# svip-lab/impersonator

Measured on NVIDIA H100. Metric: frames/sec @256x256 (per-frame inference hot path), higher is better.
Workload: dtype f16 main product + e4m3 correction products (hi/lo split), f32 accumulate

## Files before the change

impersonator_b200/csrc/conv_tc.cu:

```cuda
#include <cuda.h>

#include <stdlib.h>

#include <algorithm>
#include <new>
#include <type_traits>

#include "common.cuh"

namespace {

constexpr int TILE_H = 16, TILE_W = 8;
constexpr int SWAP_N_TILE = 64;
constexpr int SWAP_TILE_H = 32;
constexpr int KCHUNK = 64;
constexpr int ROW_BYTES = TILE_W * 128;
constexpr int MAX_TAPS = 49;
constexpr int MAX_GROUP = 8;
constexpr int RING_BYTES = 200 * 1024;
constexpr int MAX_STAGES = 8;
constexpr int NUM_CONSUMERS = 256;
constexpr int NUM_THREADS = NUM_CONSUMERS + 128;
constexpr int MAX_N_TILE = 128;
static_assert(2 * 2 * (TILE_H + MAX_GROUP - 1) * ROW_BYTES + 2 * 2 * MAX_N_TILE * 128 <= RING_BYTES,
              "every plan needs two A and two B entries in the ring");
static_assert(2 * 2 * (SWAP_TILE_H + MAX_GROUP - 1) * ROW_BYTES + 2 * 2 * SWAP_N_TILE * 128 <= RING_BYTES,
              "every swapped plan needs two A and two B entries in the ring");
static_assert(SWAP_N_TILE * (SWAP_TILE_H * TILE_W) == MAX_N_TILE * (TILE_H * TILE_W), "same accumulator budget");

__host__ __device__ constexpr int tile_rows(int n_tile) { return n_tile == SWAP_N_TILE ? SWAP_TILE_H : TILE_H; }

struct ConvParams {
    CUtensorMap a_hi[4];
    CUtensorMap a_lo[4];
    CUtensorMap w_hi;
    CUtensorMap w_lo;
    int n_img, tiles_y, tiles_x, n_tiles_n;
    int dom_h, dom_w;
    int ntaps, chunks0, chunks1;
    signed char dy[MAX_TAPS], dx[MAX_TAPS], tmap[MAX_TAPS];
    short wtap[MAX_TAPS];
    int ngroups;
    signed char g_first[MAX_TAPS], g_cnt[MAX_TAPS];
    int a_rows;
    int a_stages, b_stages;
    float* out; int out_h, out_w, cout;
    int oy_mul, oy_add, ox_mul, ox_add;
    double* stats;
    float out_scale;
    int phase_cols;
};

template <int N_TILE, bool SPLIT>
struct Cfg {
    static constexpr int B_BYTES = N_TILE * 128;
    static constexpr int B_STAGE_BYTES = B_BYTES * (SPLIT ? 2 : 1);
    static constexpr int BAR_BYTES = 4 * MAX_STAGES * 8;
    static constexpr int STATS_PARTS = N_TILE < SWAP_N_TILE ? 8 : N_TILE == SWAP_N_TILE ? 2 : 0;
    static constexpr int STATS_BYTES = STATS_PARTS * N_TILE * 8;
    static constexpr int SMEM_BYTES = 1024 + RING_BYTES + BAR_BYTES + STATS_BYTES;
    static_assert(B_STAGE_BYTES % 1024 == 0, "B entries must keep the 1024-byte swizzle alignment");
    static_assert(SMEM_BYTES <= 227 * 1024, "exceeds the shared memory of a block");
};

__device__ __forceinline__ uint32_t smem_u32(const void* p) { return (uint32_t)__cvta_generic_to_shared(p); }

__device__ __forceinline__ void mbar_init(uint64_t* bar, uint32_t count) {
    asm volatile("mbarrier.init.shared::cta.b64 [%0], %1;" ::"r"(smem_u32(bar)), "r"(count));
}
__device__ __forceinline__ void mbar_expect_tx(uint64_t* bar, uint32_t bytes) {
    asm volatile("mbarrier.arrive.expect_tx.shared::cta.b64 _, [%0], %1;" ::"r"(smem_u32(bar)), "r"(bytes) : "memory");
}
__device__ __forceinline__ void mbar_arrive(uint64_t* bar) {
    asm volatile("mbarrier.arrive.shared::cta.b64 _, [%0];" ::"r"(smem_u32(bar)) : "memory");
}
__device__ __forceinline__ bool mbar_try_wait(uint64_t* bar, uint32_t parity) {
    uint32_t ok;
    asm volatile("{\n\t.reg .pred p;\n\t"
                 "mbarrier.try_wait.parity.shared::cta.b64 p, [%1], %2;\n\t"
                 "selp.u32 %0, 1, 0, p;\n\t}"
                 : "=r"(ok) : "r"(smem_u32(bar)), "r"(parity) : "memory");
    return ok != 0;
}
__device__ __forceinline__ void mbar_wait(uint64_t* bar, uint32_t parity) {
    if (mbar_try_wait(bar, parity)) return;
    const long long t0 = clock64();
    while (!mbar_try_wait(bar, parity)) {
        if (clock64() - t0 > 4000000000ll) __trap();
    }
}
__device__ __forceinline__ bool elect_one() {
    uint32_t pred;
    asm volatile("{\n\t.reg .pred P;\n\telect.sync _|P, 0xffffffff;\n\tselp.b32 %0, 1, 0, P;\n\t}" : "=r"(pred));
    return pred != 0;
}
__device__ __forceinline__ void fence_barrier_init() { asm volatile("fence.mbarrier_init.release.cluster;" ::: "memory"); }
__device__ __forceinline__ void fence_proxy_async() { asm volatile("fence.proxy.async.shared::cta;" ::: "memory"); }

__device__ __forceinline__ void tma_load_4d(const CUtensorMap* map, void* dst, uint64_t* bar, int c0, int c1, int c2, int c3) {
    asm volatile("cp.async.bulk.tensor.4d.shared::cluster.global.mbarrier::complete_tx::bytes [%0], [%1, {%3, %4, %5, %6}], [%2];"
                 :: "r"(smem_u32(dst)), "l"(map), "r"(smem_u32(bar)), "r"(c0), "r"(c1), "r"(c2), "r"(c3) : "memory");
}
__device__ __forceinline__ void tma_load_3d(const CUtensorMap* map, void* dst, uint64_t* bar, int c0, int c1, int c2) {
    asm volatile("cp.async.bulk.tensor.3d.shared::cluster.global.mbarrier::complete_tx::bytes [%0], [%1, {%3, %4, %5}], [%2];"
                 :: "r"(smem_u32(dst)), "l"(map), "r"(smem_u32(bar)), "r"(c0), "r"(c1), "r"(c2) : "memory");
}

__device__ __forceinline__ uint64_t make_desc(uint32_t smem_addr) {
    return (uint64_t)((smem_addr & 0x3FFFF) >> 4) | (1ull << 16) | (64ull << 32) | (1ull << 62);
}
__device__ __forceinline__ void wgmma_fence() { asm volatile("wgmma.fence.sync.aligned;" ::: "memory"); }
__device__ __forceinline__ void wgmma_commit() { asm volatile("wgmma.commit_group.sync.aligned;" ::: "memory"); }
template <int N>
__device__ __forceinline__ void wgmma_wait() { asm volatile("wgmma.wait_group.sync.aligned %0;" :: "n"(N) : "memory"); }
__device__ __forceinline__ void acc_fence(float& r) { asm volatile("" : "+f"(r) :: "memory"); }

template <int N> __device__ __forceinline__ void wgmma_f16(float* d, uint64_t da, uint64_t db);
template <int N> __device__ __forceinline__ void wgmma_e4m3(float* d, uint64_t da, uint64_t db);
template <> __device__ __forceinline__ void wgmma_f16<16>(float* d, uint64_t da, uint64_t db) {
    asm volatile("{\n\t.reg .pred p;\n\tsetp.ne.b32 p, %10, 0;\n\t"
                 "wgmma.mma_async.sync.aligned.m64n16k16.f32.f16.f16 {%0, %1, %2, %3, %4, %5, %6, %7}, %8, %9, p, 1, 1, 0, 0;\n\t}"
                 : "+f"(d[0]), "+f"(d[1]), "+f"(d[2]), "+f"(d[3]), "+f"(d[4]), "+f"(d[5]), "+f"(d[6]), "+f"(d[7])
                 : "l"(da), "l"(db), "r"(1));
}
template <> __device__ __forceinline__ void wgmma_f16<32>(float* d, uint64_t da, uint64_t db) {
    asm volatile("{\n\t.reg .pred p;\n\tsetp.ne.b32 p, %18, 0;\n\t"
                 "wgmma.mma_async.sync.aligned.m64n32k16.f32.f16.f16 {%0, %1, %2, %3, %4, %5, %6, %7, %8, %9, %10, %11, %12, %13, %14, %15}, %16, %17, p, 1, 1, 0, 0;\n\t}"
                 : "+f"(d[0]), "+f"(d[1]), "+f"(d[2]), "+f"(d[3]), "+f"(d[4]), "+f"(d[5]), "+f"(d[6]), "+f"(d[7]), "+f"(d[8]), "+f"(d[9]), "+f"(d[10]), "+f"(d[11]), "+f"(d[12]), "+f"(d[13]), "+f"(d[14]), "+f"(d[15])
                 : "l"(da), "l"(db), "r"(1));
}
template <> __device__ __forceinline__ void wgmma_f16<128>(float* d, uint64_t da, uint64_t db) {
    asm volatile("{\n\t.reg .pred p;\n\tsetp.ne.b32 p, %66, 0;\n\t"
                 "wgmma.mma_async.sync.aligned.m64n128k16.f32.f16.f16 {%0, %1, %2, %3, %4, %5, %6, %7, %8, %9, %10, %11, %12, %13, %14, %15, %16, %17, %18, %19, %20, %21, %22, %23, %24, %25, %26, %27, %28, %29, %30, %31, %32, %33, %34, %35, %36, %37, %38, %39, %40, %41, %42, %43, %44, %45, %46, %47, %48, %49, %50, %51, %52, %53, %54, %55, %56, %57, %58, %59, %60, %61, %62, %63}, %64, %65, p, 1, 1, 0, 0;\n\t}"
                 : "+f"(d[0]), "+f"(d[1]), "+f"(d[2]), "+f"(d[3]), "+f"(d[4]), "+f"(d[5]), "+f"(d[6]), "+f"(d[7]), "+f"(d[8]), "+f"(d[9]), "+f"(d[10]), "+f"(d[11]), "+f"(d[12]), "+f"(d[13]), "+f"(d[14]), "+f"(d[15]), "+f"(d[16]), "+f"(d[17]), "+f"(d[18]), "+f"(d[19]), "+f"(d[20]), "+f"(d[21]), "+f"(d[22]), "+f"(d[23]), "+f"(d[24]), "+f"(d[25]), "+f"(d[26]), "+f"(d[27]), "+f"(d[28]), "+f"(d[29]), "+f"(d[30]), "+f"(d[31]), "+f"(d[32]), "+f"(d[33]), "+f"(d[34]), "+f"(d[35]), "+f"(d[36]), "+f"(d[37]), "+f"(d[38]), "+f"(d[39]), "+f"(d[40]), "+f"(d[41]), "+f"(d[42]), "+f"(d[43]), "+f"(d[44]), "+f"(d[45]), "+f"(d[46]), "+f"(d[47]), "+f"(d[48]), "+f"(d[49]), "+f"(d[50]), "+f"(d[51]), "+f"(d[52]), "+f"(d[53]), "+f"(d[54]), "+f"(d[55]), "+f"(d[56]), "+f"(d[57]), "+f"(d[58]), "+f"(d[59]), "+f"(d[60]), "+f"(d[61]), "+f"(d[62]), "+f"(d[63])
                 : "l"(da), "l"(db), "r"(1));
}
template <> __device__ __forceinline__ void wgmma_e4m3<16>(float* d, uint64_t da, uint64_t db) {
    asm volatile("{\n\t.reg .pred p;\n\tsetp.ne.b32 p, %10, 0;\n\t"
                 "wgmma.mma_async.sync.aligned.m64n16k32.f32.e4m3.e4m3 {%0, %1, %2, %3, %4, %5, %6, %7}, %8, %9, p, 1, 1;\n\t}"
                 : "+f"(d[0]), "+f"(d[1]), "+f"(d[2]), "+f"(d[3]), "+f"(d[4]), "+f"(d[5]), "+f"(d[6]), "+f"(d[7])
                 : "l"(da), "l"(db), "r"(1));
}
template <> __device__ __forceinline__ void wgmma_e4m3<32>(float* d, uint64_t da, uint64_t db) {
    asm volatile("{\n\t.reg .pred p;\n\tsetp.ne.b32 p, %18, 0;\n\t"
                 "wgmma.mma_async.sync.aligned.m64n32k32.f32.e4m3.e4m3 {%0, %1, %2, %3, %4, %5, %6, %7, %8, %9, %10, %11, %12, %13, %14, %15}, %16, %17, p, 1, 1;\n\t}"
                 : "+f"(d[0]), "+f"(d[1]), "+f"(d[2]), "+f"(d[3]), "+f"(d[4]), "+f"(d[5]), "+f"(d[6]), "+f"(d[7]), "+f"(d[8]), "+f"(d[9]), "+f"(d[10]), "+f"(d[11]), "+f"(d[12]), "+f"(d[13]), "+f"(d[14]), "+f"(d[15])
                 : "l"(da), "l"(db), "r"(1));
}
template <> __device__ __forceinline__ void wgmma_e4m3<128>(float* d, uint64_t da, uint64_t db) {
    asm volatile("{\n\t.reg .pred p;\n\tsetp.ne.b32 p, %66, 0;\n\t"
                 "wgmma.mma_async.sync.aligned.m64n128k32.f32.e4m3.e4m3 {%0, %1, %2, %3, %4, %5, %6, %7, %8, %9, %10, %11, %12, %13, %14, %15, %16, %17, %18, %19, %20, %21, %22, %23, %24, %25, %26, %27, %28, %29, %30, %31, %32, %33, %34, %35, %36, %37, %38, %39, %40, %41, %42, %43, %44, %45, %46, %47, %48, %49, %50, %51, %52, %53, %54, %55, %56, %57, %58, %59, %60, %61, %62, %63}, %64, %65, p, 1, 1;\n\t}"
                 : "+f"(d[0]), "+f"(d[1]), "+f"(d[2]), "+f"(d[3]), "+f"(d[4]), "+f"(d[5]), "+f"(d[6]), "+f"(d[7]), "+f"(d[8]), "+f"(d[9]), "+f"(d[10]), "+f"(d[11]), "+f"(d[12]), "+f"(d[13]), "+f"(d[14]), "+f"(d[15]), "+f"(d[16]), "+f"(d[17]), "+f"(d[18]), "+f"(d[19]), "+f"(d[20]), "+f"(d[21]), "+f"(d[22]), "+f"(d[23]), "+f"(d[24]), "+f"(d[25]), "+f"(d[26]), "+f"(d[27]), "+f"(d[28]), "+f"(d[29]), "+f"(d[30]), "+f"(d[31]), "+f"(d[32]), "+f"(d[33]), "+f"(d[34]), "+f"(d[35]), "+f"(d[36]), "+f"(d[37]), "+f"(d[38]), "+f"(d[39]), "+f"(d[40]), "+f"(d[41]), "+f"(d[42]), "+f"(d[43]), "+f"(d[44]), "+f"(d[45]), "+f"(d[46]), "+f"(d[47]), "+f"(d[48]), "+f"(d[49]), "+f"(d[50]), "+f"(d[51]), "+f"(d[52]), "+f"(d[53]), "+f"(d[54]), "+f"(d[55]), "+f"(d[56]), "+f"(d[57]), "+f"(d[58]), "+f"(d[59]), "+f"(d[60]), "+f"(d[61]), "+f"(d[62]), "+f"(d[63])
                 : "l"(da), "l"(db), "r"(1));
}

__device__ __forceinline__ void consumer_sync() { asm volatile("bar.sync 1, 256;" ::: "memory"); }

struct TileCoord {
    int n_idx, img, y0, x0;
};
template <int TH>
__device__ __forceinline__ TileCoord decode_tile(const ConvParams& P, int tile, int m_tiles) {
    TileCoord t;
    t.n_idx = tile / m_tiles;
    const int m_idx = tile % m_tiles;
    t.img = m_idx / (P.tiles_y * P.tiles_x);
    const int rem = m_idx % (P.tiles_y * P.tiles_x);
    t.y0 = (rem / P.tiles_x) * TH; t.x0 = (rem % P.tiles_x) * TILE_W;
    return t;
}

template <int N_TILE>
__device__ __forceinline__ void warp_tile_stats(const float* acc, bool v0, bool v1, int warp, unsigned lane, float2* s_stats)
{
#pragma unroll
    for (int j = 0; j < N_TILE / 8; j++) {
        const float a0 = v0 ? acc[4 * j] : 0.f, a1 = v0 ? acc[4 * j + 1] : 0.f;
        const float b0 = v1 ? acc[4 * j + 2] : 0.f, b1 = v1 ? acc[4 * j + 3] : 0.f;
        float s0 = a0 + b0, s1 = a1 + b1, q0 = a0 * a0 + b0 * b0, q1 = a1 * a1 + b1 * b1;
#pragma unroll
        for (int off = 4; off <= 16; off <<= 1) {
            s0 += __shfl_xor_sync(0xffffffffu, s0, off); s1 += __shfl_xor_sync(0xffffffffu, s1, off);
            q0 += __shfl_xor_sync(0xffffffffu, q0, off); q1 += __shfl_xor_sync(0xffffffffu, q1, off);
        }
        if (lane < 4) {
            s_stats[warp * N_TILE + 8 * j + 2 * lane] = make_float2(s0, q0);
            s_stats[warp * N_TILE + 8 * j + 2 * lane + 1] = make_float2(s1, q1);
        }
    }
}

template <int N_TILE, int PARTS>
__device__ __forceinline__ void flush_tile_stats(const ConvParams& P, const float2* s_stats, int img, int n_idx)
{
    consumer_sync();
    for (int col = threadIdx.x; col < N_TILE; col += NUM_CONSUMERS) {
        float s = 0.f, q = 0.f;
#pragma unroll
        for (int w = 0; w < PARTS; w++) { const float2 v = s_stats[w * N_TILE + col]; s += v.x; q += v.y; }
        int ch = n_idx * N_TILE + col;
        if (P.phase_cols > 0) ch %= P.phase_cols;
        double* dst = P.stats + 2 * ((size_t)img * P.cout + ch);
        atomicAdd(dst, (double)s);
        atomicAdd(dst + 1, (double)q);
    }
    consumer_sync();
}

template <int N_TILE>
__device__ __forceinline__ void epilogue_plain(const ConvParams& P, float* acc, const TileCoord& t, int warp, unsigned lane,
                                               float2* s_stats)
{
    const int tx = (int)(lane >> 2), x = t.x0 + tx;
    const int y[2] = {t.y0 + 2 * warp, t.y0 + 2 * warp + 1};
    const bool valid[2] = {y[0] < P.dom_h && x < P.dom_w, y[1] < P.dom_h && x < P.dom_w};
    if (P.out_scale != 1.f) {
#pragma unroll
        for (int i = 0; i < N_TILE / 2; i++) acc[i] *= P.out_scale;
    }
    if (P.out) {
        const int out_w_c = P.out_w * P.cout;
#pragma unroll
        for (int h = 0; h < 2; h++) {
            if (!valid[h]) continue;
            float* optr = P.out + (((size_t)t.img * P.out_h + (P.oy_mul * y[h] + P.oy_add)) * P.out_w + (P.ox_mul * x + P.ox_add)) * P.cout
                        + (size_t)t.n_idx * N_TILE;
#pragma unroll
            for (int j = 0; j < N_TILE / 8; j++) {
                const int c = 8 * j + 2 * (int)(lane & 3);
                float* o = optr + c;
                if (P.phase_cols > 0) {
                    const int col = t.n_idx * N_TILE + c, ph = col / P.phase_cols;
                    o = P.out + (((size_t)t.img * P.out_h + 2 * y[h]) * P.out_w + 2 * x) * P.cout
                      + (size_t)(ph >> 1) * out_w_c + (ph & 1) * P.cout + (col - ph * P.phase_cols);
                }
                *reinterpret_cast<float2*>(o) = make_float2(acc[4 * j + 2 * h], acc[4 * j + 2 * h + 1]);
            }
        }
    }
    if (P.stats) {
        warp_tile_stats<N_TILE>(acc, valid[0], valid[1], warp, lane, s_stats);
        flush_tile_stats<N_TILE, 8>(P, s_stats, t.img, t.n_idx);
    }
}

template <int N_TILE>
__device__ __forceinline__ void epilogue_channel_major(const ConvParams& P, float* acc, const TileCoord& t, int warp,
                                                       unsigned lane, float2* s_stats)
{
    const int wg = warp >> 2;
    const int c_base = N_TILE == MAX_N_TILE ? 64 * wg : 0, row0 = N_TILE == MAX_N_TILE ? 0 : 16 * wg;
    const int c0 = c_base + 16 * (warp & 3) + (int)(lane >> 2);
    const int y0 = t.y0 + row0, x0 = t.x0 + 2 * (int)(lane & 3);
    const int rows = P.dom_h - y0;
    const bool vx[2] = {x0 < P.dom_w, x0 + 1 < P.dom_w};
    const int col = t.n_idx * N_TILE + c0;
    const int ph = P.phase_cols > 0 ? col / P.phase_cols : 0;
    const int ch = col - ph * P.phase_cols;
    const size_t coff = ((size_t)(ph >> 1) * P.out_w + (ph & 1)) * P.cout + ch;
    if (P.out_scale != 1.f) {
#pragma unroll
        for (int i = 0; i < 64; i++) acc[i] *= P.out_scale;
    }
    if (P.out) {
#pragma unroll
        for (int j = 0; j < 16; j++) {
            if (j >= rows) break;
            const size_t orow = ((size_t)t.img * P.out_h + (P.oy_mul * (y0 + j) + P.oy_add)) * P.out_w;
#pragma unroll
            for (int e = 0; e < 2; e++) {
                if (!vx[e]) continue;
                float* o = P.out + (orow + (P.ox_mul * (x0 + e) + P.ox_add)) * P.cout;
                o[coff] = acc[4 * j + e];
                o[coff + 8] = acc[4 * j + 2 + e];
            }
        }
    }
    if (P.stats) {
        float s[2] = {0.f, 0.f}, q[2] = {0.f, 0.f};
#pragma unroll
        for (int j = 0; j < 16; j++) {
#pragma unroll
            for (int e = 0; e < 2; e++) {
                const bool v = j < rows && vx[e];
#pragma unroll
                for (int h = 0; h < 2; h++) {
                    const float a = v ? acc[4 * j + 2 * h + e] : 0.f;
                    s[h] += a; q[h] += a * a;
                }
            }
        }
#pragma unroll
        for (int h = 0; h < 2; h++) {
#pragma unroll
            for (int off = 1; off <= 2; off <<= 1) {
                s[h] += __shfl_xor_sync(0xffffffffu, s[h], off);
                q[h] += __shfl_xor_sync(0xffffffffu, q[h], off);
            }
        }
        if constexpr (N_TILE == SWAP_N_TILE) {
            if ((lane & 3) == 0) {
                s_stats[wg * N_TILE + c0] = make_float2(s[0], q[0]);
                s_stats[wg * N_TILE + c0 + 8] = make_float2(s[1], q[1]);
            }
            flush_tile_stats<N_TILE, 2>(P, s_stats, t.img, t.n_idx);
        } else if ((lane & 3) == 0) {
#pragma unroll
            for (int h = 0; h < 2; h++) {
                double* dst = P.stats + 2 * ((size_t)t.img * P.cout + ch + 8 * h);
                atomicAdd(dst, (double)s[h]);
                atomicAdd(dst + 1, (double)q[h]);
            }
        }
    }
}

enum { MODE_FP16 = 0, MODE_FP16X3 = 1, MODE_F8 = 2 };

template <int N_TILE, int MODE>
struct Regs {
    static constexpr int CONSUMER = N_TILE >= 64 ? (MODE == MODE_F8 ? 168 : 120) : N_TILE == 32 ? 80 : 64;
    static constexpr int LAUNCH = ((2 * CONSUMER + 40 + 2) / 3 + 7) / 8 * 8;
    static constexpr int PRODUCER = 3 * LAUNCH - 2 * CONSUMER;
    static_assert(PRODUCER >= 40 && PRODUCER % 8 == 0 && CONSUMER % 8 == 0, "setmaxnreg takes multiples of 8");
};

template <int N_TILE, bool CM>
__device__ __forceinline__ void mma_f16(float* d, uint64_t act, uint64_t w) {
    if constexpr (CM) wgmma_f16<128>(d, w, act);
    else              wgmma_f16<N_TILE>(d, act, w);
}
template <int N_TILE, bool CM>
__device__ __forceinline__ void mma_e4m3(float* d, uint64_t act, uint64_t w) {
    if constexpr (CM) wgmma_e4m3<128>(d, w, act);
    else              wgmma_e4m3<N_TILE>(d, act, w);
}

template <int N_TILE, int MODE>
__global__ void __launch_bounds__(NUM_THREADS, 1) __maxnreg__((Regs<N_TILE, MODE>::LAUNCH))
k_conv_wg(const __grid_constant__ ConvParams P)
{
    constexpr bool CM = N_TILE >= SWAP_N_TILE;
    constexpr bool SPLIT = MODE != MODE_FP16;
    constexpr int TH = N_TILE == SWAP_N_TILE ? SWAP_TILE_H : TILE_H;
    constexpr int ACC = CM ? 64 : N_TILE / 2;
    using C = Cfg<N_TILE, SPLIT>;
    extern __shared__ uint8_t smem_raw[];
    uint8_t* smem = reinterpret_cast<uint8_t*>((reinterpret_cast<uintptr_t>(smem_raw) + 1023) & ~(uintptr_t)1023);
    const int a_op_bytes = P.a_rows * ROW_BYTES;
    const int a_stage_bytes = a_op_bytes * (SPLIT ? 2 : 1);
    uint8_t* b_ring = smem + P.a_stages * a_stage_bytes;
    uint64_t* a_full = reinterpret_cast<uint64_t*>(smem + RING_BYTES);
    uint64_t* a_empty = a_full + MAX_STAGES;
    uint64_t* b_full = a_empty + MAX_STAGES;
    uint64_t* b_empty = b_full + MAX_STAGES;
    float2* s_stats = reinterpret_cast<float2*>(smem + RING_BYTES + C::BAR_BYTES);

    const int warp = threadIdx.x >> 5;
    const unsigned lane = threadIdx.x & 31;

    if (threadIdx.x == 0) {
        for (int s = 0; s < P.a_stages; s++) { mbar_init(a_full + s, 1); mbar_init(a_empty + s, NUM_CONSUMERS / 32); }
        for (int s = 0; s < P.b_stages; s++) { mbar_init(b_full + s, 1); mbar_init(b_empty + s, NUM_CONSUMERS / 32); }
        fence_barrier_init();
        fence_proxy_async();
    }
    __syncthreads();
    lwb::pdl_wait();
    lwb::pdl_trigger();

    const int nchunks = P.chunks0 + P.chunks1;
    const int m_tiles = P.n_img * P.tiles_y * P.tiles_x;
    const int total = m_tiles * P.n_tiles_n;

    if (warp >= NUM_CONSUMERS / 32) {
        asm volatile("setmaxnreg.dec.sync.aligned.u32 %0;" :: "n"(Regs<N_TILE, MODE>::PRODUCER));
        if (warp != NUM_CONSUMERS / 32) return;
        if (elect_one()) {
            asm volatile("prefetch.tensormap [%0];" :: "l"(&P.a_hi[0]) : "memory");
            asm volatile("prefetch.tensormap [%0];" :: "l"(&P.w_hi) : "memory");
            if (SPLIT) {
                asm volatile("prefetch.tensormap [%0];" :: "l"(&P.a_lo[0]) : "memory");
                asm volatile("prefetch.tensormap [%0];" :: "l"(&P.w_lo) : "memory");
            }
        }
        int as = 0, bs = 0; uint32_t aph = 0, bph = 0;
        for (int tile = blockIdx.x; tile < total; tile += gridDim.x) {
            const TileCoord t = decode_tile<TH>(P, tile, m_tiles);
            for (int g = 0; g < P.ngroups; g++) {
                const int first = P.g_first[g], cnt = P.g_cnt[g];
                const int xx = t.x0 + P.dx[first], yy = t.y0 + P.dy[first];
                for (int chunk = 0; chunk < nchunks; chunk++) {
                    const bool second = chunk >= P.chunks0;
                    const int mi = second ? 1 : P.tmap[first];
                    const int c0 = (second ? chunk - P.chunks0 : chunk) * KCHUNK;
                    mbar_wait(a_empty + as, aph ^ 1);
                    uint8_t* sa = smem + as * a_stage_bytes;
                    if (elect_one()) {
                        mbar_expect_tx(a_full + as, (uint32_t)a_stage_bytes);
                        tma_load_4d(&P.a_hi[mi], sa, a_full + as, c0, xx, yy, t.img);
                        if (SPLIT) tma_load_4d(&P.a_lo[mi], sa + a_op_bytes, a_full + as, c0, xx, yy, t.img);
                    }
                    __syncwarp();
                    if (++as == P.a_stages) { as = 0; aph ^= 1; }
                    for (int i = 0; i < cnt; i++) {
                        mbar_wait(b_empty + bs, bph ^ 1);
                        uint8_t* sb = b_ring + bs * C::B_STAGE_BYTES;
                        const int wt = P.wtap[first + i];
                        if (elect_one()) {
                            mbar_expect_tx(b_full + bs, (uint32_t)C::B_STAGE_BYTES);
                            tma_load_3d(&P.w_hi, sb, b_full + bs, chunk * KCHUNK, t.n_idx * N_TILE, wt);
                            if (SPLIT) tma_load_3d(&P.w_lo, sb + C::B_BYTES, b_full + bs, chunk * KCHUNK, t.n_idx * N_TILE, wt);
                        }
                        __syncwarp();
                        if (++bs == P.b_stages) { bs = 0; bph ^= 1; }
                    }
                }
            }
        }
    } else {
        asm volatile("setmaxnreg.inc.sync.aligned.u32 %0;" :: "n"(Regs<N_TILE, MODE>::CONSUMER));
        constexpr bool CH_SPLIT = N_TILE == MAX_N_TILE;
        const uint32_t wg = (uint32_t)(warp >> 2);
        const uint32_t a_base = smem_u32(smem) + (CH_SPLIT ? 0 : wg * (TH / 2) * ROW_BYTES);
        const uint32_t b_base = smem_u32(b_ring) + (CH_SPLIT ? wg * 64 * 128 : 0);
        float acc[ACC];
        float acc8[MODE == MODE_F8 ? ACC : 1];
        int as = 0, bs = 0; uint32_t aph = 0, bph = 0;
        for (int tile = blockIdx.x; tile < total; tile += gridDim.x) {
            const TileCoord t = decode_tile<TH>(P, tile, m_tiles);
#pragma unroll
            for (int i = 0; i < ACC; i++) acc[i] = 0.f;
#pragma unroll
            for (int i = 0; i < (MODE == MODE_F8 ? ACC : 1); i++) acc8[i] = 0.f;
            int prev_b = -1, prev_a = -1;
            for (int g = 0; g < P.ngroups; g++) {
                const int cnt = P.g_cnt[g];
                for (int chunk = 0; chunk < nchunks; chunk++) {
                    mbar_wait(a_full + as, aph);
                    const uint32_t a_hi = a_base + as * a_stage_bytes;
                    for (int i = 0; i < cnt; i++) {
                        mbar_wait(b_full + bs, bph);
                        const uint32_t ai = a_hi + i * ROW_BYTES, al = ai + a_op_bytes;
                        const uint32_t b_hi = b_base + bs * C::B_STAGE_BYTES, b_lo = b_hi + C::B_BYTES;
                        wgmma_fence();
#pragma unroll
                        for (int k = 0; k < KCHUNK / 16; k++) {
                            const uint64_t da = make_desc(ai + k * 32), db = make_desc(b_hi + k * 32);
                            mma_f16<N_TILE, CM>(acc, da, db);
                            if constexpr (MODE == MODE_F8) {
                                mma_e4m3<N_TILE, CM>(acc8, make_desc(al + k * 32), make_desc(b_lo + k * 32));
                            } else if constexpr (MODE == MODE_FP16X3) {
                                mma_f16<N_TILE, CM>(acc, da, make_desc(b_lo + k * 32));
                                mma_f16<N_TILE, CM>(acc, make_desc(al + k * 32), db);
                            }
                        }
                        wgmma_commit();
                        if (prev_b >= 0) {
                            wgmma_wait<1>();
                            if (lane == 0) {
                                mbar_arrive(b_empty + prev_b);
                                if (prev_a >= 0) mbar_arrive(a_empty + prev_a);
                            }
                            prev_a = -1;
                        }
                        prev_b = bs;
                        if (++bs == P.b_stages) { bs = 0; bph ^= 1; }
                    }
                    prev_a = as;
                    if (++as == P.a_stages) { as = 0; aph ^= 1; }
                }
            }
            wgmma_wait<0>();
#pragma unroll
            for (int i = 0; i < ACC; i++) acc_fence(acc[i]);
            if constexpr (MODE == MODE_F8) {
#pragma unroll
                for (int i = 0; i < ACC; i++) { acc_fence(acc8[i]); acc[i] += acc8[i]; }
            }
            if (lane == 0) { mbar_arrive(b_empty + prev_b); mbar_arrive(a_empty + prev_a); }
            if constexpr (CM) epilogue_channel_major<N_TILE>(P, acc, t, warp, lane, s_stats);
            else              epilogue_plain<N_TILE>(P, acc, t, warp, lane, s_stats);
        }
    }
}

typedef CUresult (*EncodeTiledFn)(CUtensorMap*, CUtensorMapDataType, cuuint32_t, void*, const cuuint64_t*,
                                  const cuuint64_t*, const cuuint32_t*, const cuuint32_t*, CUtensorMapInterleave,
                                  CUtensorMapSwizzle, CUtensorMapL2promotion, CUtensorMapFloatOOBfill);

EncodeTiledFn get_encode()
{
    static EncodeTiledFn fn = nullptr;
    if (!fn) {
        void* p = nullptr;
        cudaDriverEntryPointQueryResult q;
        if (cudaGetDriverEntryPoint("cuTensorMapEncodeTiled", &p, cudaEnableDefault, &q) != cudaSuccess || !p) return nullptr;
        fn = (EncodeTiledFn)p;
    }
    return fn;
}

int encode_map(CUtensorMap* m, const void* base, int rank, const uint64_t* dims, const uint64_t* strides_bytes, const uint32_t* box)
{
    EncodeTiledFn enc = get_encode();
    if (!enc) { lwb::set_error("cuTensorMapEncodeTiled entry point not available"); return LWB_E_CUDA; }
    cuuint64_t gdim[5]; cuuint64_t gstr[4]; cuuint32_t bx[5]; cuuint32_t es[5];
    for (int i = 0; i < rank; i++) { gdim[i] = dims[i]; bx[i] = box[i]; es[i] = 1; }
    for (int i = 0; i < rank - 1; i++) gstr[i] = strides_bytes[i];
    CUresult r = enc(m, CU_TENSOR_MAP_DATA_TYPE_FLOAT16, (cuuint32_t)rank, const_cast<void*>(base), gdim, gstr, bx, es,
                     CU_TENSOR_MAP_INTERLEAVE_NONE, CU_TENSOR_MAP_SWIZZLE_128B, CU_TENSOR_MAP_L2_PROMOTION_L2_256B,
                     CU_TENSOR_MAP_FLOAT_OOB_FILL_NONE);
    if (r != CUDA_SUCCESS) {
        lwb::set_error("cuTensorMapEncodeTiled failed (%d): rank %d dims [%llu,%llu,%llu,%llu] strides [%llu,%llu,%llu] box [%u,%u,%u,%u]",
                       (int)r, rank, (unsigned long long)dims[0], (unsigned long long)dims[1], (unsigned long long)(rank > 2 ? dims[2] : 0),
                       (unsigned long long)(rank > 3 ? dims[3] : 0), (unsigned long long)strides_bytes[0],
                       (unsigned long long)(rank > 2 ? strides_bytes[1] : 0), (unsigned long long)(rank > 3 ? strides_bytes[2] : 0),
                       box[0], box[1], rank > 2 ? box[2] : 0, rank > 3 ? box[3] : 0);
        return LWB_E_CUDA;
    }
    return LWB_OK;
}

struct Launch {
    ConvParams p;
    int n_tile;
    int mode;
    int grid;
};

template <int N_TILE, int MODE>
int launch_wg(const Launch& L, cudaStream_t st)
{
    using C = Cfg<N_TILE, MODE != MODE_FP16>;
    static bool attr_set_dev[lwb::kMaxDevices] = {};
    bool& attr_set = attr_set_dev[lwb::device_slot()];
    if (!attr_set) {
        LWB_CUDA_OK(cudaFuncSetAttribute(k_conv_wg<N_TILE, MODE>, cudaFuncAttributeMaxDynamicSharedMemorySize, C::SMEM_BYTES));
        attr_set = true;
    }
    LWB_CUDA_OK(lwb::launch_pdl(k_conv_wg<N_TILE, MODE>, dim3(L.grid), dim3(NUM_THREADS), C::SMEM_BYTES, st, L.p));
    LWB_LAUNCH_OK();
    return LWB_OK;
}

template <class F>
int with_instance(int n_tile, int mode, F&& f)
{
    auto modes = [&](auto nt) {
        if (mode == MODE_F8) return f(nt, std::integral_constant<int, MODE_F8>());
        if (mode == MODE_FP16X3) return f(nt, std::integral_constant<int, MODE_FP16X3>());
        return f(nt, std::integral_constant<int, MODE_FP16>());
    };
    switch (n_tile) {
        case 16:  return modes(std::integral_constant<int, 16>());
        case 32:  return modes(std::integral_constant<int, 32>());
        case 64:  return modes(std::integral_constant<int, 64>());
        case 128: return modes(std::integral_constant<int, 128>());
    }
    lwb::set_error("conv_tc: unsupported N tile %d", n_tile);
    return LWB_E_UNSUPPORTED;
}

int launch(const Launch& L, cudaStream_t st)
{
    return with_instance(L.n_tile, L.mode,
                         [&](auto nt, auto md) { return launch_wg<decltype(nt)::value, decltype(md)::value>(L, st); });
}

int pick_n_tile(int cout, int forced)
{
    if (forced > 0) return forced > MAX_N_TILE && forced % MAX_N_TILE == 0 ? MAX_N_TILE : forced;
    if (cout % 128 == 0) return 128;
    if (cout % 64 == 0) return 64;
    if (cout % 32 == 0) return 32;
    if (cout % 16 == 0) return 16;
    return -1;
}

struct View {
    const uint16_t* hi;
    const uint16_t* lo;
    uint64_t dims[4], str[3];
};

struct LaunchSpec {
    int ntaps;
    signed char dy[MAX_TAPS], dx[MAX_TAPS], tmap[MAX_TAPS];
    short wtap[MAX_TAPS];
    int chunks0, chunks1;
    int nviews;
    View a[4];
    View w;
    int ncols;
    int dom_h, dom_w;
    int oy_mul, oy_add, ox_mul, ox_add, phase_cols;
    int n_tile;

    void tap(int y, int x, int view, int wt)
    {
        dy[ntaps] = (signed char)y; dx[ntaps] = (signed char)x; tmap[ntaps] = (signed char)view; wtap[ntaps] = (short)wt;
        ntaps++;
    }
};

}

struct lwb_conv_plan {
    int num;
    Launch launches[4];
};

static View nhwc_view(const uint16_t* hi, const uint16_t* lo, int n, int h, int w, int c, int step = 1, int py = 0, int px = 0)
{
    const size_t off = ((size_t)py * w + px) * c;
    return View{hi + off, lo ? lo + off : lo,
                {(uint64_t)c, (uint64_t)((w - px + step - 1) / step), (uint64_t)((h - py + step - 1) / step), (uint64_t)n},
                {(uint64_t)step * c * 2, (uint64_t)step * w * c * 2, (uint64_t)h * w * c * 2}};
}

static View weight_view(const uint16_t* hi, const uint16_t* lo, int k, int ncols, int taps)
{
    return View{hi, lo, {(uint64_t)k, (uint64_t)ncols, (uint64_t)taps}, {(uint64_t)k * 2, (uint64_t)ncols * k * 2}};
}

static int encode_pair(CUtensorMap* hi, CUtensorMap* lo, int rank, const View& v, const uint32_t* box, bool split)
{
    const int rc = encode_map(hi, v.hi, rank, v.dims, v.str, box);
    return rc != LWB_OK || !split ? rc : encode_map(lo, v.lo, rank, v.dims, v.str, box);
}

static void group_taps(ConvParams& p, int tile_h)
{
    int order[MAX_TAPS];
    for (int t = 0; t < p.ntaps; t++) order[t] = t;
    std::stable_sort(order, order + p.ntaps, [&](int a, int b) {
        if (p.tmap[a] != p.tmap[b]) return p.tmap[a] < p.tmap[b];
        if (p.dx[a] != p.dx[b]) return p.dx[a] < p.dx[b];
        return p.dy[a] < p.dy[b];
    });
    const ConvParams src = p;
    int longest = 0;
    p.ngroups = 0;
    for (int t = 0; t < p.ntaps; t++) {
        const int o = order[t];
        p.dy[t] = src.dy[o]; p.dx[t] = src.dx[o]; p.tmap[t] = src.tmap[o]; p.wtap[t] = src.wtap[o];
        const bool joins = t > 0 && p.tmap[t] == p.tmap[t - 1] && p.dx[t] == p.dx[t - 1] && p.dy[t] == p.dy[t - 1] + 1 &&
                           p.g_cnt[p.ngroups - 1] < MAX_GROUP;
        if (!joins) { p.g_first[p.ngroups] = (signed char)t; p.g_cnt[p.ngroups] = 0; p.ngroups++; }
        p.g_cnt[p.ngroups - 1]++;
        longest = std::max(longest, (int)p.g_cnt[p.ngroups - 1]);
    }
    p.a_rows = tile_h + longest - 1;
}

static void pick_rings(ConvParams& p, int n_tile, bool split)
{
    const int ops = split ? 2 : 1;
    const int a_bytes = p.a_rows * ROW_BYTES * ops, b_bytes = n_tile * 128 * ops;
    const int longest = p.a_rows - tile_rows(n_tile) + 1;
    int best = 0;
    for (int a = 2; a <= MAX_STAGES; a++) {
        const int b = std::min(MAX_STAGES, (RING_BYTES - a * a_bytes) / b_bytes);
        if (b < 2) break;
        if (std::min(a * longest, b) > best) { best = std::min(a * longest, b); p.a_stages = a; p.b_stages = b; }
    }
}

static int build_launch(Launch& L, const LaunchSpec& s, const lwb_conv_desc* d, float* out_raw, double* stats, int sms)
{
    const bool split = d->split != 0;
    ConvParams& p = L.p;
    memset(&p, 0, sizeof(p));
    p.ntaps = s.ntaps; p.chunks0 = s.chunks0; p.chunks1 = s.chunks1;
    for (int t = 0; t < s.ntaps; t++) { p.dy[t] = s.dy[t]; p.dx[t] = s.dx[t]; p.tmap[t] = s.tmap[t]; p.wtap[t] = s.wtap[t]; }
    group_taps(p, tile_rows(s.n_tile));
    int rc;
    const uint32_t a_box[4] = {KCHUNK, TILE_W, (uint32_t)p.a_rows, 1};
    for (int v = 0; v < s.nviews; v++)
        if ((rc = encode_pair(&p.a_hi[v], &p.a_lo[v], 4, s.a[v], a_box, split)) != LWB_OK) return rc;
    const uint32_t w_box[3] = {KCHUNK, (uint32_t)s.n_tile, 1};
    if ((rc = encode_pair(&p.w_hi, &p.w_lo, 3, s.w, w_box, split)) != LWB_OK) return rc;
    p.n_img = d->n;
    p.dom_h = s.dom_h; p.dom_w = s.dom_w;
    p.tiles_y = lwb::ceil_div(s.dom_h, tile_rows(s.n_tile)); p.tiles_x = lwb::ceil_div(s.dom_w, TILE_W);
    p.n_tiles_n = s.ncols / s.n_tile;
    p.out = out_raw; p.out_h = d->h_out; p.out_w = d->w_out; p.cout = d->cout;
    p.oy_mul = s.oy_mul; p.oy_add = s.oy_add; p.ox_mul = s.ox_mul; p.ox_add = s.ox_add; p.phase_cols = s.phase_cols;
    p.stats = stats;
    p.out_scale = ldexpf(1.f, -d->w_exp);
    L.n_tile = s.n_tile; L.mode = d->split;
    pick_rings(p, s.n_tile, split);
    const long total = (long)p.n_img * p.tiles_y * p.tiles_x * p.n_tiles_n;
    L.grid = (int)(total < sms ? total : sms);
    return LWB_OK;
}

extern "C" int lwb_conv_plan_create(const lwb_conv_desc* d,
                                    const uint16_t* x0_hi, const uint16_t* x0_lo,
                                    const uint16_t* x1_hi, const uint16_t* x1_lo,
                                    const uint16_t* w_hi, const uint16_t* w_lo,
                                    float* out_raw, double* stats, lwb_conv_plan** plan_out)
{
    LWB_CHECK_ARG(d && x0_hi && w_hi && out_raw && plan_out, "null pointer");
    const bool split = d->split != 0;
    const bool f8 = d->split == 2;
    LWB_CHECK_ARG(d->split >= 0 && d->split <= 2, "split must be 0, 1 or 2");
    LWB_CHECK_ARG(!split || (x0_lo && w_lo), "split mode needs the lo operands");
    LWB_CHECK_ARG(!f8 || (!d->rowk && !d->halo), "the fp8 lo mode is not available for row-K / halo plans");
    LWB_CHECK_ARG(d->n > 0 && d->h_in > 0 && d->w_in > 0 && d->cout > 0, "non-positive size");
    LWB_CHECK_ARG(d->cout % 16 == 0, "cout must be a multiple of 16");
    LWB_CHECK_ARG(d->w_exp >= -40 && d->w_exp <= 60, "w_exp out of range");
    const int n_tile = pick_n_tile(d->cout, d->n_tile);
    LWB_CHECK_ARG(n_tile > 0 && d->cout % n_tile == 0, "no N tile divides cout");
    if (d->halo) {
        LWB_CHECK_ARG(d->stride == 1 && !d->transposed && d->dil == 1, "halo mode needs stride 1, dilation 1, not transposed");
        if (d->rowk) LWB_CHECK_ARG(d->kw <= 8 && d->cin0 == 8 && d->cin1 == 0 && d->row_pitch >= d->w_in + 8, "row-K shape");
        else         LWB_CHECK_ARG(d->kw <= 9 && (d->kw & 1) && (d->kh & 1), "halo mode needs an odd kernel, kw <= 9, with 'same' padding (kh/2, kw/2)");
    }

    const int sms = lwb::sm_count();

    LaunchSpec s = {};
    s.n_tile = n_tile; s.ncols = d->cout;
    s.dom_h = d->h_out; s.dom_w = d->w_out;
    s.oy_mul = s.ox_mul = 1;
    s.nviews = 1;
    LaunchSpec specs[4];
    int num = 1;
    if (d->rowk) {
        LWB_CHECK_ARG(d->stride == 1 && !d->transposed && d->kw <= 8 && d->cin0 == 8 && d->cin1 == 0, "row-K needs stride 1, kw <= 8, 8 channels");
        LWB_CHECK_ARG(d->h_out == d->h_in && d->w_out == d->w_in && d->row_pitch >= d->w_in + 8, "row-K shape");
        for (int ky = 0; ky < d->kh; ky++) s.tap(ky, 0, 0, ky);
        s.chunks0 = 1;
        const uint64_t hp = d->h_in + d->kh - 1, row_bytes = (uint64_t)d->row_pitch * 16;
        s.a[0] = View{x0_hi, x0_lo, {64, (uint64_t)d->w_in, hp, (uint64_t)d->n}, {16, row_bytes, hp * row_bytes}};
        s.w = weight_view(w_hi, w_lo, 64, d->cout, d->kh);
    } else {
        LWB_CHECK_ARG(d->cin0 % KCHUNK == 0 && d->cin1 % KCHUNK == 0 && d->cin0 > 0, "input channels must be multiples of 64");
        LWB_CHECK_ARG(d->cin1 == 0 || (x1_hi && (!split || x1_lo)), "second input missing");
        const int cin_total = d->cin0 + d->cin1;
        const int ntaps_w = d->kh * d->kw;
        LWB_CHECK_ARG(ntaps_w <= MAX_TAPS, "too many filter taps");
        s.chunks0 = d->cin0 / KCHUNK; s.chunks1 = d->cin1 / KCHUNK;
        s.a[0] = nhwc_view(x0_hi, x0_lo, d->n, d->h_in, d->w_in, d->cin0);
        s.w = weight_view(w_hi, w_lo, cin_total, d->cout, ntaps_w);
        if (d->transposed) {
            LWB_CHECK_ARG(d->kh == 3 && d->kw == 3 && d->stride == 2 && d->pad == 1 && d->cin1 == 0, "transposed conv: only k3 s2 p1 op1");
            LWB_CHECK_ARG(d->h_out == 2 * d->h_in && d->w_out == 2 * d->w_in, "transposed conv output must be 2x input");
            s.dom_h = d->h_in; s.dom_w = d->w_in;
            s.oy_mul = s.ox_mul = 2;
        }
        if (d->transposed == 2) {
            s.n_tile = MAX_N_TILE;
            s.ncols = 4 * d->cout;
            LWB_CHECK_ARG(d->cout % 32 == 0 && s.ncols % s.n_tile == 0, "merged transposed conv needs cout in multiples of 32");
            for (int t = 0; t < 4; t++) s.tap(t >> 1, t & 1, 0, t);
            s.w = weight_view(w_hi, w_lo, cin_total, s.ncols, 4);
            s.phase_cols = d->cout;
        } else if (d->transposed) {
            const int ky_list[2][2] = {{1, -1}, {2, 0}}, d_list[2][2] = {{0, 0}, {0, 1}}, cnt[2] = {1, 2};
            num = 4;
            for (int a = 0; a < 2; a++) for (int b = 0; b < 2; b++) {
                LaunchSpec& q = specs[a * 2 + b];
                q = s;
                for (int i = 0; i < cnt[a]; i++) for (int j = 0; j < cnt[b]; j++)
                    q.tap(d_list[a][i], d_list[b][j], 0, ky_list[a][i] * 3 + ky_list[b][j]);
                q.oy_add = a; q.ox_add = b;
            }
        } else {
            LWB_CHECK_ARG(d->stride == 1 || d->stride == 2, "stride must be 1 or 2");
            LWB_CHECK_ARG(d->stride == 1 || d->cin1 == 0, "concat input only with stride 1");
            const int st = d->stride;
            for (int ky = 0; ky < d->kh; ky++) for (int kx = 0; kx < d->kw; kx++) {
                const int oy = ky * d->dil - d->pad, ox = kx * d->dil - (d->pad_w >= 0 ? d->pad_w : d->pad);
                if (oy < -127 || oy > 127 || ox < -127 || ox > 127) { lwb::set_error("conv_tc: tap offset out of range"); return LWB_E_UNSUPPORTED; }
                const int py = ((oy % st) + st) % st, px = ((ox % st) + st) % st;
                s.tap((oy - py) / st, (ox - px) / st, py * 2 + px, s.ntaps);
            }
            s.nviews = st * st;
            for (int v = 0; v < s.nviews; v++) s.a[v] = nhwc_view(x0_hi, x0_lo, d->n, d->h_in, d->w_in, d->cin0, st, v >> 1, v & 1);
            if (d->cin1) {
                s.nviews = 2;
                s.a[1] = nhwc_view(x1_hi, x1_lo, d->n, d->h_in, d->w_in, d->cin1);
            }
        }
    }
    if (num == 1) specs[0] = s;

    lwb_conv_plan* plan = new (std::nothrow) lwb_conv_plan();
    LWB_CHECK_ARG(plan, "out of host memory");
    for (; plan->num < num; plan->num++) {
        const int rc = build_launch(plan->launches[plan->num], specs[plan->num], d, out_raw, stats, sms);
        if (rc != LWB_OK) { delete plan; return rc; }
    }
    *plan_out = plan;
    return LWB_OK;
}

extern "C" int lwb_conv_plan_run(const lwb_conv_plan* plan, lwb_stream_t stream)
{
    LWB_CHECK_ARG(plan, "null plan");
    for (int i = 0; i < plan->num; i++) {
        const int rc = launch(plan->launches[i], (cudaStream_t)stream);
        if (rc != LWB_OK) return rc;
    }
    return LWB_OK;
}

extern "C" void lwb_conv_plan_destroy(lwb_conv_plan* plan) { delete plan; }

extern "C" int lwb_conv_plan_num_launches(const lwb_conv_plan* plan) { return plan ? plan->num : 0; }

extern "C" int lwb_conv2d_nhwc(const lwb_conv_desc* d,
                               const uint16_t* x0_hi, const uint16_t* x0_lo,
                               const uint16_t* x1_hi, const uint16_t* x1_lo,
                               const uint16_t* w_hi, const uint16_t* w_lo,
                               float* out_raw, double* stats, lwb_stream_t stream)
{
    lwb_conv_plan* plan = nullptr;
    int rc = lwb_conv_plan_create(d, x0_hi, x0_lo, x1_hi, x1_lo, w_hi, w_lo, out_raw, stats, &plan);
    if (rc != LWB_OK) return rc;
    rc = lwb_conv_plan_run(plan, stream);
    lwb_conv_plan_destroy(plan);
    return rc;
}

template <int N_TILE, int MODE>
static int conv_resources(int* out)
{
    using C = Cfg<N_TILE, MODE != MODE_FP16>;
    cudaFuncAttributes a;
    LWB_CUDA_OK(cudaFuncSetAttribute(k_conv_wg<N_TILE, MODE>, cudaFuncAttributeMaxDynamicSharedMemorySize, C::SMEM_BYTES));
    LWB_CUDA_OK(cudaFuncGetAttributes(&a, k_conv_wg<N_TILE, MODE>));
    int blocks = 0;
    LWB_CUDA_OK(cudaOccupancyMaxActiveBlocksPerMultiprocessor(&blocks, k_conv_wg<N_TILE, MODE>, NUM_THREADS, C::SMEM_BYTES));
    out[0] = a.numRegs; out[1] = (int)a.sharedSizeBytes; out[2] = C::SMEM_BYTES; out[3] = (int)a.localSizeBytes;
    out[4] = NUM_THREADS; out[5] = blocks; out[6] = Regs<N_TILE, MODE>::CONSUMER;
    return LWB_OK;
}

extern "C" int lwb_conv_kernel_resources(int n_tile, int mode, int* out)
{
    LWB_CHECK_ARG(out, "null pointer");
    LWB_CHECK_ARG(mode >= 0 && mode <= 2, "mode must be 0, 1 or 2");
    return with_instance(n_tile, mode,
                         [&](auto nt, auto md) { return conv_resources<decltype(nt)::value, decltype(md)::value>(out); });
}
```

Measured before the change: 2278.

## Skip structurally-zero taps per N tile in merged transposed conv

For the merged transposed conv, each N tile covers a subset of output phases, and only the taps those phases actually use are now loaded and multiplied. This adds per-N-tile tap sets with their own groupings and a second, shorter TMA box so groups with fewer rows load less data. Tile order changes so N is the fastest-varying index, which puts neighbouring N tiles of the same spatial tile on adjacent blocks. The costs are a larger parameter struct, extra tensor maps and more complex producer bookkeeping.

```diff
diff --git a/impersonator_b200/csrc/conv_tc.cu b/impersonator_b200/csrc/conv_tc.cu
--- a/impersonator_b200/csrc/conv_tc.cu
+++ b/impersonator_b200/csrc/conv_tc.cu
@@ -16,6 +16,7 @@
 constexpr int KCHUNK = 64;
 constexpr int ROW_BYTES = TILE_W * 128;
 constexpr int MAX_TAPS = 49;
+constexpr int MAX_TAP_SETS = 4;
 constexpr int MAX_GROUP = 8;
 constexpr int RING_BYTES = 200 * 1024;
 constexpr int MAX_STAGES = 8;
@@ -31,8 +32,8 @@
 __host__ __device__ constexpr int tile_rows(int n_tile) { return n_tile == SWAP_N_TILE ? SWAP_TILE_H : TILE_H; }
 
 struct ConvParams {
-    CUtensorMap a_hi[4];
-    CUtensorMap a_lo[4];
+    CUtensorMap a_hi[2][4];
+    CUtensorMap a_lo[2][4];
     CUtensorMap w_hi;
     CUtensorMap w_lo;
     int n_img, tiles_y, tiles_x, n_tiles_n;
@@ -40,9 +41,12 @@
     int ntaps, chunks0, chunks1;
     signed char dy[MAX_TAPS], dx[MAX_TAPS], tmap[MAX_TAPS];
     short wtap[MAX_TAPS];
-    int ngroups;
-    signed char g_first[MAX_TAPS], g_cnt[MAX_TAPS];
+    int tap_sets;
+    int ngroups[MAX_TAP_SETS];
+    signed char g_first[MAX_TAP_SETS][MAX_TAPS], g_cnt[MAX_TAP_SETS][MAX_TAPS];
+    signed char g_box[MAX_TAP_SETS][MAX_TAPS];
     int a_rows;
+    int box_rows[2];
     int a_stages, b_stages;
     float* out; int out_h, out_w, cout;
     int oy_mul, oy_add, ox_mul, ox_add;
@@ -50,6 +54,7 @@
     float out_scale;
     int phase_cols;
 };
+static_assert(sizeof(ConvParams) <= 4096, "ConvParams is passed as a __grid_constant__ kernel parameter (4 KB)");
 
 template <int N_TILE, bool SPLIT>
 struct Cfg {
@@ -160,10 +165,10 @@
     int n_idx, img, y0, x0;
 };
 template <int TH>
-__device__ __forceinline__ TileCoord decode_tile(const ConvParams& P, int tile, int m_tiles) {
+__device__ __forceinline__ TileCoord decode_tile(const ConvParams& P, int tile) {
     TileCoord t;
-    t.n_idx = tile / m_tiles;
-    const int m_idx = tile % m_tiles;
+    t.n_idx = tile % P.n_tiles_n;
+    const int m_idx = tile / P.n_tiles_n;
     t.img = m_idx / (P.tiles_y * P.tiles_x);
     const int rem = m_idx % (P.tiles_y * P.tiles_x);
     t.y0 = (rem / P.tiles_x) * TH; t.x0 = (rem % P.tiles_x) * TILE_W;
@@ -370,26 +375,27 @@
     lwb::pdl_trigger();
 
     const int nchunks = P.chunks0 + P.chunks1;
-    const int m_tiles = P.n_img * P.tiles_y * P.tiles_x;
-    const int total = m_tiles * P.n_tiles_n;
+    const int total = P.n_img * P.tiles_y * P.tiles_x * P.n_tiles_n;
 
     if (warp >= NUM_CONSUMERS / 32) {
         asm volatile("setmaxnreg.dec.sync.aligned.u32 %0;" :: "n"(Regs<N_TILE, MODE>::PRODUCER));
         if (warp != NUM_CONSUMERS / 32) return;
         if (elect_one()) {
-            asm volatile("prefetch.tensormap [%0];" :: "l"(&P.a_hi[0]) : "memory");
+            asm volatile("prefetch.tensormap [%0];" :: "l"(&P.a_hi[0][0]) : "memory");
             asm volatile("prefetch.tensormap [%0];" :: "l"(&P.w_hi) : "memory");
             if (SPLIT) {
-                asm volatile("prefetch.tensormap [%0];" :: "l"(&P.a_lo[0]) : "memory");
+                asm volatile("prefetch.tensormap [%0];" :: "l"(&P.a_lo[0][0]) : "memory");
                 asm volatile("prefetch.tensormap [%0];" :: "l"(&P.w_lo) : "memory");
             }
         }
         int as = 0, bs = 0; uint32_t aph = 0, bph = 0;
         for (int tile = blockIdx.x; tile < total; tile += gridDim.x) {
-            const TileCoord t = decode_tile<TH>(P, tile, m_tiles);
-            for (int g = 0; g < P.ngroups; g++) {
-                const int first = P.g_first[g], cnt = P.g_cnt[g];
+            const TileCoord t = decode_tile<TH>(P, tile);
+            const int ts = P.tap_sets > 1 ? t.n_idx : 0;
+            for (int g = 0; g < P.ngroups[ts]; g++) {
+                const int first = P.g_first[ts][g], cnt = P.g_cnt[ts][g], box = P.g_box[ts][g];
                 const int xx = t.x0 + P.dx[first], yy = t.y0 + P.dy[first];
+                const uint32_t box_bytes = (uint32_t)(P.box_rows[box] * ROW_BYTES * (SPLIT ? 2 : 1));
                 for (int chunk = 0; chunk < nchunks; chunk++) {
                     const bool second = chunk >= P.chunks0;
                     const int mi = second ? 1 : P.tmap[first];
@@ -397,9 +403,9 @@
                     mbar_wait(a_empty + as, aph ^ 1);
                     uint8_t* sa = smem + as * a_stage_bytes;
                     if (elect_one()) {
-                        mbar_expect_tx(a_full + as, (uint32_t)a_stage_bytes);
-                        tma_load_4d(&P.a_hi[mi], sa, a_full + as, c0, xx, yy, t.img);
-                        if (SPLIT) tma_load_4d(&P.a_lo[mi], sa + a_op_bytes, a_full + as, c0, xx, yy, t.img);
+                        mbar_expect_tx(a_full + as, box_bytes);
+                        tma_load_4d(&P.a_hi[box][mi], sa, a_full + as, c0, xx, yy, t.img);
+                        if (SPLIT) tma_load_4d(&P.a_lo[box][mi], sa + a_op_bytes, a_full + as, c0, xx, yy, t.img);
                     }
                     __syncwarp();
                     if (++as == P.a_stages) { as = 0; aph ^= 1; }
@@ -428,14 +434,15 @@
         float acc8[MODE == MODE_F8 ? ACC : 1];
         int as = 0, bs = 0; uint32_t aph = 0, bph = 0;
         for (int tile = blockIdx.x; tile < total; tile += gridDim.x) {
-            const TileCoord t = decode_tile<TH>(P, tile, m_tiles);
+            const TileCoord t = decode_tile<TH>(P, tile);
 #pragma unroll
             for (int i = 0; i < ACC; i++) acc[i] = 0.f;
 #pragma unroll
             for (int i = 0; i < (MODE == MODE_F8 ? ACC : 1); i++) acc8[i] = 0.f;
             int prev_b = -1, prev_a = -1;
-            for (int g = 0; g < P.ngroups; g++) {
-                const int cnt = P.g_cnt[g];
+            const int ts = P.tap_sets > 1 ? t.n_idx : 0;
+            for (int g = 0; g < P.ngroups[ts]; g++) {
+                const int cnt = P.g_cnt[ts][g];
                 for (int chunk = 0; chunk < nchunks; chunk++) {
                     mbar_wait(a_full + as, aph);
                     const uint32_t a_hi = a_base + as * a_stage_bytes;
@@ -596,6 +603,8 @@
     int dom_h, dom_w;
     int oy_mul, oy_add, ox_mul, ox_add, phase_cols;
     int n_tile;
+    int tap_sets;
+    uint64_t tap_mask[MAX_TAP_SETS];
 
     void tap(int y, int x, int view, int wt)
     {
@@ -630,7 +639,7 @@
     return rc != LWB_OK || !split ? rc : encode_map(lo, v.lo, rank, v.dims, v.str, box);
 }
 
-static void group_taps(ConvParams& p, int tile_h)
+static void group_taps(ConvParams& p, int tile_h, int sets, const uint64_t* masks)
 {
     int order[MAX_TAPS];
     for (int t = 0; t < p.ntaps; t++) order[t] = t;
@@ -640,18 +649,36 @@
         return p.dy[a] < p.dy[b];
     });
     const ConvParams src = p;
-    int longest = 0;
-    p.ngroups = 0;
     for (int t = 0; t < p.ntaps; t++) {
         const int o = order[t];
         p.dy[t] = src.dy[o]; p.dx[t] = src.dx[o]; p.tmap[t] = src.tmap[o]; p.wtap[t] = src.wtap[o];
-        const bool joins = t > 0 && p.tmap[t] == p.tmap[t - 1] && p.dx[t] == p.dx[t - 1] && p.dy[t] == p.dy[t - 1] + 1 &&
-                           p.g_cnt[p.ngroups - 1] < MAX_GROUP;
-        if (!joins) { p.g_first[p.ngroups] = (signed char)t; p.g_cnt[p.ngroups] = 0; p.ngroups++; }
-        p.g_cnt[p.ngroups - 1]++;
-        longest = std::max(longest, (int)p.g_cnt[p.ngroups - 1]);
-    }
+    }
+    p.tap_sets = sets;
+    int longest = 0, shortest = MAX_GROUP;
+    for (int s = 0; s < sets; s++) {
+        int& ng = p.ngroups[s];
+        ng = 0;
+        bool prev_in = false;
+        for (int t = 0; t < p.ntaps; t++) {
+            const bool in = (masks[s] >> order[t]) & 1;
+            const bool joins = in && prev_in && p.tmap[t] == p.tmap[t - 1] && p.dx[t] == p.dx[t - 1] &&
+                               p.dy[t] == p.dy[t - 1] + 1 && p.g_cnt[s][ng - 1] < MAX_GROUP;
+            prev_in = in;
+            if (!in) continue;
+            if (!joins) { p.g_first[s][ng] = (signed char)t; p.g_cnt[s][ng] = 0; ng++; }
+            p.g_cnt[s][ng - 1]++;
+        }
+        for (int g = 0; g < ng; g++) {
+            longest = std::max(longest, (int)p.g_cnt[s][g]);
+            shortest = std::min(shortest, (int)p.g_cnt[s][g]);
+        }
+    }
+    for (int s = 0; s < sets; s++)
+        for (int g = 0; g < p.ngroups[s]; g++)
+            p.g_box[s][g] = (signed char)(p.g_cnt[s][g] == shortest && shortest < longest);
     p.a_rows = tile_h + longest - 1;
+    p.box_rows[0] = p.a_rows;
+    p.box_rows[1] = tile_h + shortest - 1;
 }
 
 static void pick_rings(ConvParams& p, int n_tile, bool split)
@@ -674,17 +701,21 @@
     memset(&p, 0, sizeof(p));
     p.ntaps = s.ntaps; p.chunks0 = s.chunks0; p.chunks1 = s.chunks1;
     for (int t = 0; t < s.ntaps; t++) { p.dy[t] = s.dy[t]; p.dx[t] = s.dx[t]; p.tmap[t] = s.tmap[t]; p.wtap[t] = s.wtap[t]; }
-    group_taps(p, tile_rows(s.n_tile));
+    const uint64_t all_taps = (1ull << s.ntaps) - 1;
+    group_taps(p, tile_rows(s.n_tile), s.tap_sets > 0 ? s.tap_sets : 1, s.tap_sets > 0 ? s.tap_mask : &all_taps);
     int rc;
-    const uint32_t a_box[4] = {KCHUNK, TILE_W, (uint32_t)p.a_rows, 1};
-    for (int v = 0; v < s.nviews; v++)
-        if ((rc = encode_pair(&p.a_hi[v], &p.a_lo[v], 4, s.a[v], a_box, split)) != LWB_OK) return rc;
+    for (int b = 0; b < (p.box_rows[1] < p.box_rows[0] ? 2 : 1); b++) {
+        const uint32_t a_box[4] = {KCHUNK, TILE_W, (uint32_t)p.box_rows[b], 1};
+        for (int v = 0; v < s.nviews; v++)
+            if ((rc = encode_pair(&p.a_hi[b][v], &p.a_lo[b][v], 4, s.a[v], a_box, split)) != LWB_OK) return rc;
+    }
     const uint32_t w_box[3] = {KCHUNK, (uint32_t)s.n_tile, 1};
     if ((rc = encode_pair(&p.w_hi, &p.w_lo, 3, s.w, w_box, split)) != LWB_OK) return rc;
     p.n_img = d->n;
     p.dom_h = s.dom_h; p.dom_w = s.dom_w;
     p.tiles_y = lwb::ceil_div(s.dom_h, tile_rows(s.n_tile)); p.tiles_x = lwb::ceil_div(s.dom_w, TILE_W);
     p.n_tiles_n = s.ncols / s.n_tile;
+    if (p.tap_sets > 1 && p.tap_sets != p.n_tiles_n) { lwb::set_error("conv_tc: one tap set per N tile"); return LWB_E_UNSUPPORTED; }
     p.out = out_raw; p.out_h = d->h_out; p.out_w = d->w_out; p.cout = d->cout;
     p.oy_mul = s.oy_mul; p.oy_add = s.oy_add; p.ox_mul = s.ox_mul; p.ox_add = s.ox_add; p.phase_cols = s.phase_cols;
     p.stats = stats;
@@ -758,6 +789,16 @@
             for (int t = 0; t < 4; t++) s.tap(t >> 1, t & 1, 0, t);
             s.w = weight_view(w_hi, w_lo, cin_total, s.ncols, 4);
             s.phase_cols = d->cout;
+            const int ntn = s.ncols / s.n_tile;
+            if (ntn > 1 && ntn <= MAX_TAP_SETS) {
+                s.tap_sets = ntn;
+                for (int n = 0; n < ntn; n++) {
+                    s.tap_mask[n] = 0;
+                    for (int ph = n * s.n_tile / d->cout; ph <= ((n + 1) * s.n_tile - 1) / d->cout; ph++)
+                        for (int t = 0; t < 4; t++)
+                            if ((t >> 1) <= (ph >> 1) && (t & 1) <= (ph & 1)) s.tap_mask[n] |= 1ull << t;
+                }
+            }
         } else if (d->transposed) {
             const int ky_list[2][2] = {{1, -1}, {2, 0}}, d_list[2][2] = {{0, 0}, {0, 1}}, cnt[2] = {1, 2};
             num = 4;
```

Result: faster. 2345 (median of 6 runs) (+2.9%).
